# actionml/universal-recommender

Measured on AMD Instinct MI355X. Metric: cooccurrence pairs/sec (A'A+A'B) + LLR top-k items/sec, higher is better.
Workload: dtype int32 counts / f64 LLR; 1 GPU; config4: synthetic 10M users x 2M items, Zipf-1.0, 5 event types (purchase/view/add-to-cart/search/category-pref); generator=torch Philox on the GPU (universal_recommender_amd.synth.generate_device), maxEventsPerEventType=500, maxCorrelatorsPerEventType=50, seed=20260925, entry_point=urcco_context_build_device (C ABI, include/urcco.h), launch=one process per GPU, parallelism=items range-partitioned over 1 GPU(s), one HIP stream per event type

## Files before the change

### universal-recommender_amd/csrc/cco_expand.hip

```cpp
#include "cco_kernels.h"

#include <atomic>
#include <cstdio>
#include <cstdlib>

#include "cco_common.h"
#include "cco_device.h"


namespace urcco {

__global__ __launch_bounds__(256) void item_entropy_kernel(const int32_t* __restrict__ counts, int32_t n, long long n_users,
                                                           double* __restrict__ ent, double* __restrict__ xlx_n) {
  const int64_t i = (int64_t)blockIdx.x * 256 + threadIdx.x;
  if (i < n) {
    const long long c = counts[i];
    ent[i] = entropy2(c, n_users - c);
  }
  if (i == 0 && xlx_n) *xlx_n = x_log_x(n_users);
}

hipError_t launch_item_entropy(hipStream_t st, const int32_t* counts, int32_t n, long long n_users, double* ent, double* xlx_n) {
  const int blocks = n > 0 ? (n + 255) / 256 : 1;
  hipLaunchKernelGGL(item_entropy_kernel, dim3(blocks), dim3(256), 0, st, counts, n, n_users, ent, xlx_n);
  return hipGetLastError();
}

__global__ __launch_bounds__(256) void narrow_counts_kernel(const int32_t* __restrict__ counts, int64_t n, unsigned short* __restrict__ out16,
                                                            int32_t* __restrict__ bad) {
  int over = 0;
  for (int64_t i = (int64_t)blockIdx.x * 256 + threadIdx.x; i < n; i += (int64_t)gridDim.x * 256) {
    const int c = counts[i];
    out16[i] = (unsigned short)c;
    over += (c < 0 || c > 0xffff) ? 1 : 0;
  }
  if (over) atomicAdd(bad, over);
}
hipError_t launch_narrow_counts(hipStream_t st, int n_cu, const int32_t* counts, int64_t n, unsigned short* out16, int32_t* bad) {
  hipError_t e = hipMemsetAsync(bad, 0, sizeof(int32_t), st);
  if (e != hipSuccess || n <= 0) return e;
  int64_t blocks = (n + 255) / 256;
  if (blocks > (int64_t)n_cu * 8) blocks = (int64_t)n_cu * 8;
  hipLaunchKernelGGL(narrow_counts_kernel, dim3((unsigned)blocks), dim3(256), 0, st, counts, n, out16, bad);
  return hipGetLastError();
}

typedef int urcco_v4i __attribute__((ext_vector_type(4)));
// ... 400 lines not shown
```

### universal-recommender_amd/csrc/cco_kernels.h

```cpp
#pragma once
#include <hip/hip_runtime.h>
#include <stdint.h>

namespace urcco {

constexpr int NBINS = 7;
constexpr int MP_KMAX_HOST = 256;

constexpr int SCAN_TILE = 2048;
constexpr int DS_TILE = 4096;
constexpr int GLOBAL_BIN_BLOCKS = 128;
constexpr int BIN_TILE = 1024;
constexpr int XLX_TABLE_HOST = 4096;
constexpr int BIN_COLS_HOST = 3 * NBINS + 3;
constexpr int BIN_OFF_LEN = NBINS + 3;
constexpr int CAND_SLOTS = 64;
constexpr int STATS_LEN = 32;

constexpr int32_t DBG_GATHER_ONLY = 1;
constexpr int32_t DBG_NO_LLR = 2;
constexpr int32_t DBG_NO_TOPK = 4;
constexpr int32_t DBG_NO_SELECT = 8;
constexpr int32_t DBG_NO_RANK = 16;
constexpr int32_t DBG_NO_COUNT_GATHER = 512;
constexpr int32_t DBG_UNFUSED_EXPAND = 4096;
constexpr int32_t DBG_GATHERED_PRIMARY = 8192;
constexpr int32_t DBG_UNFILTERED_EXCHANGE = 16384;
constexpr int32_t DBG_SELECT_DELAY = 131072;
constexpr int32_t DBG_UNPACKED_COUNTS = 1048576;
constexpr int32_t DBG_ROW_KERNELS = DBG_GATHER_ONLY | DBG_NO_LLR | DBG_NO_TOPK | DBG_NO_SELECT | DBG_NO_RANK | DBG_NO_COUNT_GATHER | DBG_SELECT_DELAY;

constexpr int32_t FORM_WIDE = 1;
constexpr int32_t FORM_PS64 = 2;
constexpr int32_t FORM_TILE = 4;
constexpr int32_t FORM_PACK = 8;
constexpr int32_t FORM_HOST = 16;
constexpr unsigned long long NARROW_LIMIT = 1ull << 32;
struct ExpandForm {
  int32_t* word;
  const int32_t* pack_bad;
  int32_t host_wide;
  int32_t host_narrow;
  unsigned long long limit;
  long long seed;
};

struct CcoArgs {
  const int32_t* bin_rows;
  const int32_t* bin_off;
  const int64_t* a_col_ptr;
  const unsigned* pstart32;
  const int64_t* wp;
// ... 14 lines not shown
  int32_t debug;
  long long n_users;
  int32_t n_cols_b;
  int32_t item_lo;
  int32_t exclude_self;
  int32_t k;
  int32_t has_min_llr;
  double min_llr;
  int32_t count_bits;
  int32_t col_bytes;
  int32_t g_log2;
  int32_t unordered;
  int32_t* out_count;
  int32_t* out_idx;
  double* out_llr;
  unsigned long long* err;
  unsigned long long* cand;
  int32_t* g_counts;
  unsigned long long* g_cand_key;
  int32_t* g_cand_col;
  int32_t g_blocks;
  const int64_t* pstart64;
  const int64_t* work;
};

hipError_t launch_column_counts(hipStream_t st, int n_cu, const int32_t* col_idx, int64_t nnz, int32_t n_cols, int32_t* counts);
constexpr int64_t PH_MIN_NNZ = 1 << 20;
int64_t column_counts_scratch_bytes(int64_t nnz, int32_t n_cols);
hipError_t launch_column_counts_partitioned(hipStream_t st, const int32_t* col_idx, int64_t nnz, const int64_t* nnz_dev, int32_t n_cols,
                                            int32_t* counts, char* scratch);

hipError_t launch_scan_i32(hipStream_t st, const int32_t* in, int64_t n, int64_t* out, int64_t* tile_sums);
hipError_t launch_slice_weights(hipStream_t st, const unsigned short* loc_t, int n_buckets, int64_t n_parts, long long* weight);

hipError_t launch_downsample_flags(hipStream_t st, int n_cu, int64_t n_rows, const int64_t* row_ptr, const int32_t* col_idx, int64_t nnz,
                                   int32_t n_cols, const int32_t* raw_counts, unsigned long long* thresholds, uint32_t seed, int32_t max_n,
                                   int row_rate_mode, int64_t row_base, int64_t* tile_rows, unsigned long long* flags, int64_t* tile_count,
                                   int32_t* post_counts);
hipError_t launch_downsample_scan(hipStream_t st, int64_t nnz, int64_t* tile_count);
hipError_t launch_downsample_compact(hipStream_t st, int64_t n_rows, const int64_t* row_ptr, const int32_t* col_idx, int64_t nnz,
                                     const int64_t* tile_rows, const unsigned long long* flags, const int64_t* tile_off, int64_t* out_row_ptr,
                                     int32_t* out_col_idx);

hipError_t launch_scan_i32_range(hipStream_t st, const int32_t* in, int64_t n, int32_t lo, int32_t hi, int64_t* out, int64_t* tile_sums);
hipError_t launch_transpose(hipStream_t st, int n_cu, int64_t n_rows, const int64_t* row_ptr, const int32_t* col_idx, int g_log2,
                            const int64_t* col_ptr, int32_t* cursor, int32_t* out_row_idx, int32_t col_lo, int32_t col_hi);
// ... 25 lines not shown
hipError_t launch_need_mask(hipStream_t st, int n_cu, int64_t n_rows, const int64_t* a_row_ptr, const int32_t* a_col_idx, const int32_t* bounds, int world,
                            unsigned long long* mask);
hipError_t launch_masked_lengths(hipStream_t st, int n_cu, int64_t n_rows, const int64_t* row_ptr, const unsigned long long* mask, int world, int32_t* mlen, int64_t* off,
                                 int64_t* tile_sums, int64_t* to_nnz);
hipError_t launch_pack_rows(hipStream_t st, int n_cu, int64_t n_rows, const int64_t* row_ptr, const int32_t* col_idx, const unsigned long long* mask, int world,
                            const int64_t* off, int32_t* pack);
hipError_t launch_scan_u16(hipStream_t st, const unsigned short* in, int64_t n, int64_t* out, int64_t* tile_sums);
hipError_t launch_frag_record(hipStream_t st, int32_t world, const int32_t* bounds, const int64_t* l_cp, const int32_t* bad, int64_t* rec);
hipError_t launch_frag_place(hipStream_t st, int n_cu, int32_t world, int32_t lo, int32_t n_range, const void* lens, int wire16, const int64_t* src_off,
                             const int32_t* ents, const int64_t* a_cp, const int64_t* sizes, int32_t* a_ri);

hipError_t launch_validate_csr(hipStream_t st, int n_cu, int64_t n_rows, const int64_t* row_ptr, const int32_t* col_idx, int64_t nnz, int32_t n_cols,
                               int g_log2, int64_t rp0, unsigned long long* err);
hipError_t launch_rebase_i64(hipStream_t st, int n_cu, int64_t* p, int64_t n, int64_t delta);
hipError_t launch_publish_word(hipStream_t st, const unsigned long long* src, unsigned long long* dst_mapped);

hipError_t launch_pop_counts(hipStream_t st, int n_cu, int64_t n, const int32_t* item, const int64_t* t_ms, int32_t n_items, int n_buckets,
                             const int64_t* bounds, int32_t* counts);

hipError_t launch_pack_counts(hipStream_t st, int n_cu, const int32_t* col_idx, const int64_t* nnz_dev, int64_t nnz_bound, const unsigned short* counts16,
                              const int32_t* bad16, int32_t count_bits, int32_t* out, int32_t* bad);
hipError_t launch_xlx_table(hipStream_t st, double* tab);
hipError_t launch_xlx_hi_table(hipStream_t st, double* tab , const double* xlx_tab, long long n_users);
hipError_t launch_item_entropy(hipStream_t st, const int32_t* counts, int32_t n, long long n_users, double* ent, double* xlx_n);
hipError_t launch_narrow_counts(hipStream_t st, int n_cu, const int32_t* counts, int64_t n, unsigned short* out16, int32_t* bad);

hipError_t launch_expand_prepare(hipStream_t st, int n_cu, const int64_t* a_col_ptr, int32_t n_items_a, const int32_t* a_row_idx,
                                 const int64_t* b_row_ptr, unsigned* b_rp32_scratch , int64_t n_rows_b, int64_t cap,
                                 unsigned* pstart32, int64_t* pstart64, int32_t* plen, int64_t* wp, int64_t* tile_sums, ExpandForm form);
constexpr int EXPAND_MULTI_MAX = 8;
hipError_t launch_expand_prepare_multi(hipStream_t st, int n_cu, const int64_t* a_col_ptr, int32_t n_items_a, const int32_t* a_row_idx, int n,
                                       const int64_t* const* b_row_ptr, int64_t n_rows_b, int64_t cap, unsigned* const* pstart, int32_t* const* plen, void* T,
                                       int64_t* const* tsum );
hipError_t launch_expand_scan(hipStream_t st, const int64_t* a_col_ptr, int32_t n_items_a, const int32_t* plen, int64_t cap, int64_t* wp, int64_t* tile_sums,
                              bool tile_sums_ready, const unsigned* pstart32, int64_t* pstart64, ExpandForm form);
hipError_t launch_row_work(hipStream_t st, int n_cu, int32_t item_lo, int32_t item_hi, const int64_t* a_col_ptr, const int64_t* wp, const int64_t* tile_sums,
                           const int32_t* form, int64_t* work);

hipError_t launch_binning(hipStream_t st, int32_t item_lo, int32_t n, const int64_t* work, const int32_t* cnt_a, int32_t n_cols_b,
                          int32_t count_bits, int32_t k, int64_t* tile_counts, int32_t* bin_off, int32_t* bin_rows, int64_t* stats);

hipError_t launch_cco_rows_bin(hipStream_t st, int n_cu, const CcoArgs& args, int bin, int32_t n_rows );
hipError_t launch_bin_out_stats(hipStream_t st, const int32_t* bin_rows, const int32_t* bin_off, int32_t item_lo, const int32_t* out_count,
                                const unsigned long long* cand, int64_t* stats);

hipError_t launch_compact_indicators(hipStream_t st, int32_t n_rows, int32_t k, const int32_t* count, const int32_t* idx,
                                     const double* llr, const int64_t* row_ptr, int32_t* out_idx, double* out_llr);
// ... 99 lines not shown
```

### universal-recommender_amd/csrc/cco_rows.hip

```cpp
#include "cco_kernels.h"

#include <atomic>
#include <cstdlib>

#include "cco_common.h"
#include "cco_device.h"


namespace urcco {

constexpr int E0 = 1024, E1S = 4096, E1 = 8192, E2S = 16384, E2 = 32768;
constexpr int MP_KMAX = 256;

__host__ __device__ constexpr int table_slots(int E, int T) { return (2 * E / 3) / (2 * T) * (2 * T); }
constexpr int URCCO_WB1 = 512;
constexpr int URCCO_WB2 = 8192;
__device__ __forceinline__ int choose_bin(long long w, long long ca, int32_t n_cols_b, int32_t count_bits, int32_t k) {
  if (ca <= 0 || w <= 0) return -1;
  if (count_bits < 31 && ca > ((1ll << count_bits) - 1)) return NBINS - 1;
  if (w <= 64 && ca <= 64) return 0;
  int cap_bin = NBINS - 1;
  const long long dmax = (w < (long long)n_cols_b ? w : (long long)n_cols_b) * 3 + (long long)k * 3 + 2;
  if (dmax <= E0) cap_bin = 1;
  else if (dmax <= E1S) cap_bin = 2;
// ... 391 lines not shown
template <int T>
__device__ __forceinline__ unsigned claim_positions(bool want, unsigned* counter, unsigned& wave_count) {
  const unsigned long long m = __ballot(want);
  const unsigned c = (unsigned)__popcll(m);
  unsigned base;
  if (T == WAVE) {
    base = wave_count;
    wave_count += c;
  } else {
    unsigned b = 0u;
    if ((threadIdx.x & (WAVE - 1)) == 0 && c != 0u) b = atomicAdd(counter, c);
    base = wave_read_lane(b, 0);
  }
  return base + lanes_below(m);
}
template <int T>
__device__ __forceinline__ unsigned team_exclusive_scan(unsigned v, unsigned* s_wsum , unsigned* total) {
  const int lane = threadIdx.x & (WAVE - 1);
  const unsigned inc = wave_inclusive_sum(v);
  if (T == WAVE) {
    *total = wave_read_lane(inc, WAVE - 1);
    return inc - v;
  }
  const int wave = (threadIdx.x % T) / WAVE;
  if (lane == WAVE - 1) s_wsum[wave] = inc;
  __syncthreads();
  unsigned base = 0, tot = 0;
#pragma unroll
  for (int w = 0; w < T / WAVE; ++w) {
    const unsigned sw = s_wsum[w];
    if (w < wave) base += sw;
    tot += sw;
  }
  __syncthreads();
  *total = tot;
  return base + inc - v;
}

constexpr int URCCO_U_WAVE = 2;
constexpr int URCCO_U_BS = 2;
constexpr int URCCO_U_B = 2;
constexpr int URCCO_U_H = 1;
constexpr int URCCO_U_C = 1;
constexpr int URCCO_OCC_WAVE = 8;
constexpr int URCCO_OCC_BS = 7;
constexpr int URCCO_G_WAVE = 2;
constexpr int URCCO_SEL_AMB_WAVE = 64;
constexpr int URCCO_SEL_AMB_BLOCK = 128;
constexpr int URCCO_G_BLOCK = 2;
constexpr int URCCO_SEL_M_BLOCK = 128;
constexpr int URCCO_G_CU = 2;
template <bool NARROW> struct PStart { typedef int64_t type; };
template <> struct PStart<true> { typedef unsigned type; };
template <int T, int E, int U, bool MP = false, bool DBG = false, bool PK = false>
__global__ __launch_bounds__((T < 256 ? 256 : T), (T == 64 ? URCCO_OCC_WAVE : (T == 256 && E == 4096 ? URCCO_OCC_BS : (T == 512 ? 4 : 1)))) void cco_rows_kernel(CcoArgs a, int bin) {
  if ((a.b_packed != nullptr && (a.pk_known != 0 || *a.form == 0)) != PK) return;
  using PS = typename PStart<PK>::type;
  constexpr int WS = PK ? 1 : 2;
  const int dbg = DBG ? a.debug : 0;
  constexpr bool packed = PK;
  URCCO_OWN_GLOBAL_PTR(const int32_t, b_col_idx, PK ? a.b_packed : a.b_col_idx);
  const int cshift = 32 - a.count_bits;
  const unsigned colmask = PK ? (1u << cshift) - 1u : a.b_col_mask;
  URCCO_OWN_GLOBAL_PTR(const unsigned short, cnt_b16, a.cnt_b16);
  URCCO_OWN_GLOBAL_PTR(const int32_t, cnt_b, a.cnt_b);
  URCCO_OWN_GLOBAL_PTR(const double, xlx_tab, a.xlx_tab);
  URCCO_OWN_GLOBAL_PTR(const double, xlx_hi, a.xlx_hi);
  URCCO_OWN_GLOBAL_PTR(const double, col_ent, a.col_ent);
  URCCO_OWN_GLOBAL_PTR(int32_t, out_idx, a.out_idx);
  URCCO_OWN_GLOBAL_PTR(double, out_llr, a.out_llr);
  long long n_users = a.n_users;
  URCCO_OWN_SGPRS(n_users);
  constexpr int BLOCK = T < 256 ? 256 : T;
  constexpr int TEAMS = BLOCK / T;
  constexpr int SH = table_slots(E, T);
  constexpr int SPT = SH / T;
  static_assert(SH % (2 * T) == 0 && SH + SH / 2 <= E && SH <= 65536, "slots and the candidate list share the table; a slot index takes 16 bits of a list word");
  constexpr unsigned CAND_CAP = (unsigned)(E - SH);
// ... 27 lines not shown
  __shared__ unsigned long long s_selthr[TEAMS * 2];
  constexpr bool SKIP_SHARED = T >= 256;
  __shared__ unsigned long long s_kbits[2 * NW];
  __shared__ unsigned s_mpflag;
  __shared__ unsigned s_ncand;
  __shared__ unsigned long long s_runk[MP ? 2 * MP_KMAX : 1];
  __shared__ unsigned s_runc[MP ? 2 * MP_KMAX : 1];

  const int team = TEAMS == 1 ? 0 : uni((int)threadIdx.x / T);
  const int tl = threadIdx.x % T;
  const int lane = threadIdx.x & (WAVE - 1);
  unsigned* tab = s_tab + team * E;
  unsigned* cand = tab + SH;
  unsigned long long* share = s_share + (SHARE ? team * SHARE_WORDS : 0);
  PS* ustart = reinterpret_cast<PS*>(SHARE ? reinterpret_cast<long long*>(share) : s_ustart + team * T);
  unsigned* uoff = SHARE ? reinterpret_cast<unsigned*>(share + T) : s_uoff + team * (T + 1);
  unsigned* hist = SHARE ? reinterpret_cast<unsigned*>(share) : s_hist + team * NH * 128;
  unsigned* sel_res = s_selres + team * 4;
  unsigned* nsel = sel_res + 3;
  unsigned short* lst = SHARE ? reinterpret_cast<unsigned short*>(share) + SH_LST / 2 : s_lst + team * (SEL_CAP > 0 ? SEL_CAP : 1);
  unsigned long long* amb_key = SHARE ? share : s_ambkey + team * SEL_M;
  unsigned* amb_col = SHARE ? reinterpret_cast<unsigned*>(share + SEL_M) : s_ambcol + team * SEL_M;
  unsigned long long* sel_thr = s_selthr + team * 2;
  const int list_start = a.bin_off[bin];
  const int list_n = a.bin_off[bin + 1] - list_start;
  const int total_teams = gridDim.x * TEAMS;
  bool ident = (long long)a.n_cols_b * 3 + (long long)a.k * 3 + 2 <= E && a.n_cols_b <= SH;
  int cb = a.count_bits;
  unsigned cmask = (1u << cb) - 1u;
  unsigned long long cand_acc = 0ull;
  const double xlx_n = *a.xlx_n;
  const bool use16 = *a.cnt16_bad == 0;

  int li = blockIdx.x * TEAMS + team;
  if (li >= list_n) return;
  const int S = total_teams;
  auto pos_of = [&](int l) { return list_start + (l < list_n ? l : list_n - 1); };
  const unsigned* wp32 = reinterpret_cast<const unsigned*>(a.wp);
  const PS* pstart;
  if constexpr (PK) pstart = a.pstart32;
  else pstart = a.pstart64;
  const int lane3 = lane < 3 ? lane : 2;
  int idv = a.bin_rows[pos_of(li + lane3 * S)];
  int64_t cs_c, ce_c;
  int64_t bnd_b;
  {
// ... 47 lines not shown
        const long long cols_pp = ((long long)a.n_cols_b + (1ll << mp_s) - 1) >> mp_s;
        int kb = 1;
        while ((1ll << kb) <= cols_pp) ++kb;
        const bool count_ok = kb <= 1 || ca_row <= (1ll << (32 - kb)) - 1;
        const long long exp_d = ((dd >> mp_s) + (dd >> (mp_s + 2)) + 1) < cols_pp ? ((dd >> mp_s) + (dd >> (mp_s + 2)) + 1) : cols_pp;
        if (count_ok && exp_d <= cap) break;
      }
    }
  mp_again:
    if (MP) {
      const long long cols_pp = ((long long)a.n_cols_b + (1ll << mp_s) - 1) >> mp_s;
      int kb = 1;
      while ((1ll << kb) <= cols_pp) ++kb;
      cb = 32 - kb;
      cmask = cb >= 32 ? 0xffffffffu : (1u << cb) - 1u;
      ident = cols_pp * 3 + 3ll * a.k + 2ll <= (long long)E && cols_pp <= (long long)SH;
      if (tl == 0) s_mpflag = 0u;
    }
    const unsigned mp_mask = MP ? (1u << mp_s) - 1u : 0u;
#pragma unroll
    for (int q = 0; q < SPT / 2; ++q) *reinterpret_cast<uint2*>(&tab[2 * (tl + q * T)]) = make_uint2(0u, 0u);
    unsigned n_cand = 0u;
    if (T != WAVE && tl == 0) s_ncand = 0u;
    team_sync<T>();
    for (int64_t c0 = cs; c0 < ce; c0 += T) {
      const int64_t c1 = c0 + T < ce ? c0 + T : ce;
      const bool pre = !MP && c0 == cs;
      const unsigned w0 = pre ? row_w0 : uni(wp32[WS * c0]);
      const unsigned total = (pre ? row_w1 : uni(wp32[WS * c1])) - w0;
      const int64_t p = c0 + tl;
      if (p < c1) {
        ustart[tl] = pre ? my_start : pstart[p];
        uoff[tl] = (pre ? my_wp : wp32[WS * p]) - w0;
      } else {
        uoff[tl] = total;
      }
      if (tl == 0) uoff[T] = total;
      team_sync<T>();
      if (total > 0u) {
        const unsigned per = (total + T - 1) / T;
        const unsigned first = (unsigned)tl * per;
        const bool act = first < total;
        const unsigned last = act ? (first + per < total ? first + per : total) : first;
        int o = 0;
        int64_t pos = 0;
        unsigned uend = 0u;
// ... 56 lines not shown
              n_cand += n_new;
            } else {
              unsigned b = 0u;
              if (lane == 0) b = atomicAdd(&s_ncand, n_new);
              base = wave_read_lane(b, 0);
            }
#pragma unroll
            for (int q = 0; q < G; ++q) {
              const unsigned idx = base + lanes_below(cm[q]);
              if (at[q] != ~0u) {
                if (idx < CAND_CAP) cand[idx] = at[q] | ((packed ? jj[q] >> cshift : 0u) << 16);
                else if (MP) s_mpflag = 1u;
                else atomicAdd(a.err, 1ull);
              }
              base += (unsigned)__popcll(cm[q]);
            }
          }
        }
      }
      team_sync<T>();
    }
    unsigned D = T == WAVE ? n_cand : uni(s_ncand);
    if (D > CAND_CAP) D = CAND_CAP;
    {
      unsigned cw[CPT], cv[CPT];
#pragma unroll
      for (int q = 0; q < CPT; ++q) {
        const unsigned t = (unsigned)tl + (unsigned)q * T;
        cw[q] = 0u;
        cv[q] = 0u;
        if (t < D) {
          cw[q] = cand[t];
          cv[q] = tab[cw[q] & 0xffffu];
        }
      }
      team_sync<T>();
      unsigned long long* kk0 = reinterpret_cast<unsigned long long*>(tab + ((D + 1u) & ~1u));
      const bool fits = !MP || 3ll * D + 3ll * a.k + 2ll <= (long long)E;
#pragma unroll
      for (int q = 0; q < CPT; ++q) {
        const unsigned t = (unsigned)tl + (unsigned)q * T;
        if (t < D) {
          tab[t] = cv[q];
          if (fits) kk0[t] = (unsigned long long)(cw[q] >> 16);
        }
      }
    }
    team_sync<T>();
    if (MP) {
      if (s_mpflag != 0u || 3ll * D + 3ll * a.k + 2ll > (long long)E) {
        team_sync<T>();
        ++mp_s;
        mp_q = 0u;
        n_run = 0u;
        goto mp_again;
      }
    }
    cand_acc += D;
    unsigned long long* kk = reinterpret_cast<unsigned long long*>(tab + ((D + 1u) & ~1u));
    unsigned n_valid = 0;
    unsigned long long kand = ~0ull, kor = 0ull;
    {
      const long long ca = a.cnt_a[i];
      const double row_entropy = a.ent_a[i];
      for (unsigned base = 0; base < D; base += U * T) {
        const unsigned t0 = base + (unsigned)tl;
        unsigned vv[U];
        int cbj[U];
// ... 22 lines not shown
            if (!(a.exclude_self && j == i)) {
              const double llr = all_in_tables ? llr_from_tables(row_entropy, xlx_n, (unsigned)k11, (unsigned)ca, (unsigned)cbj[x], xlx_tab, xlx_hi, col_ent)
                                               : ((dbg & DBG_NO_LLR) ? (double)k11
                                                            : llr_of(row_entropy, xlx_n, k11, ca, (long long)cbj[x], n_users, xlx_tab, xlx_hi, col_ent));
              if (llr > 0.0 && (!a.has_min_llr || llr >= a.min_llr)) key = (unsigned long long)__double_as_longlong(llr);
            }
            kk[t] = key;
            if (key != 0ull) {
              ++n_valid;
              if (SKIP_SHARED) {
                kand &= key;
                kor |= key;
              }
            }
          }
        }
      }
    }
    URCCO_SETTLE(idv); URCCO_SETTLE(bnd_c);
    if (!MP) { URCCO_SETTLE(pf_w0); URCCO_SETTLE(pf_w1); URCCO_SETTLE(pf_wp); URCCO_SETTLE(pf_start); }
    if (SKIP_SHARED) {
      wave_and_or_u64(kand, kor);
      if (lane == 0) {
        s_kbits[2 * (tl / WAVE)] = kand;
        s_kbits[2 * (tl / WAVE) + 1] = kor;
      }
    }
    unsigned C;
    team_exclusive_scan<T>(n_valid, s_wsum, &C);
    C = uni(C);
    team_sync<T>();
    const int64_t obase = ((int64_t)(i - a.item_lo)) * a.k;
    unsigned long long thr_key = 0ull;
    unsigned thr_ncol = 0u;
    bool row_done = false;
    if (!(dbg & DBG_NO_TOPK)) {
      if (dbg & DBG_NO_SELECT) {
        if (C > (unsigned)a.k) thr_key = ~0ull;
      } else if (C > (unsigned)a.k) {
        unsigned need = (unsigned)a.k;
        if (a.col_bytes < 4) thr_ncol = 0xffffffffu << (8 * a.col_bytes);
        int p0 = 0;
        if (!SKIP_SHARED) {
          kand = ~0ull;
          kor = 0ull;
          for (unsigned base = 0; base < D; base += T) {
            const unsigned t = base + (unsigned)tl;
            const unsigned long long key = t < D ? kk[t] : 0ull;
// ... 726 lines not shown
#pragma unroll
      for (int w2 = 0; w2 < NW; ++w2) {
        const unsigned long long ok = s_pkey[r & 1][w2];
        const int oc = s_pcol[r & 1][w2];
        if (best_before(ok, oc, wk, wc)) {
          wk = ok;
          wc = oc;
        }
      }
      if (wk == 0ull) break;
      if (threadIdx.x == 0) {
        a.out_idx[obase + r] = wc;
        a.out_llr[obase + r] = __longlong_as_double((long long)wk);
      }
      last_key = wk;
      last_col = wc;
      ++emitted;
    }
    if (threadIdx.x == 0) a.out_count[i - a.item_lo] = emitted;
    __syncthreads();
  }
}

static int blocks_per_cu(int bin) {
  static std::atomic<int> cache[7];
  if (cache[bin].load(std::memory_order_relaxed) == 0) {
    int n = 0;
    hipError_t e = hipErrorUnknown;
    if (bin == 0) e = hipOccupancyMaxActiveBlocksPerMultiprocessor(&n, (cco_rows_micro_kernel<WAVE, false, false>), 256, 0);
    if (bin == 1) e = hipOccupancyMaxActiveBlocksPerMultiprocessor(&n, cco_rows_kernel<64, E0, URCCO_U_WAVE>, 256, 0);
    if (bin == 2) e = hipOccupancyMaxActiveBlocksPerMultiprocessor(&n, cco_rows_kernel<256, E1S, URCCO_U_BS>, 256, 0);
    if (bin == 3) e = hipOccupancyMaxActiveBlocksPerMultiprocessor(&n, cco_rows_kernel<256, E1, URCCO_U_B>, 256, 0);
    if (bin == 4) e = hipOccupancyMaxActiveBlocksPerMultiprocessor(&n, cco_rows_kernel<512, E2S, URCCO_U_H>, 512, 0);
    if (bin == 5) e = hipOccupancyMaxActiveBlocksPerMultiprocessor(&n, cco_rows_kernel<1024, E2, URCCO_U_C>, 1024, 0);
    if (bin == 6) e = hipOccupancyMaxActiveBlocksPerMultiprocessor(&n, cco_rows_kernel<1024, E2, URCCO_U_C, true>, 1024, 0);
    cache[bin].store((e == hipSuccess && n > 0) ? n : 1, std::memory_order_relaxed);
  }
  return cache[bin].load(std::memory_order_relaxed);
}

hipError_t launch_cco_rows_bin(hipStream_t st, int n_cu, const CcoArgs& args, int bin, int32_t n_rows) {
  static constexpr int factor[NBINS] = {8, 8, 8, 8, 4, 4, 2};
  constexpr int micro_factor32 = 3, micro_factor16 = 2;
  auto grid = [&](int b, int f = 0) {
    const long long fill = (long long)n_cu * blocks_per_cu(b);
    const long long teams = b <= 1 ? 4 : 1;
    long long cap = ((long long)n_rows + teams * 32 - 1) / (teams * 32);
    if (cap < 2 * fill) cap = 2 * fill;
    long long blocks = fill * (f > 0 ? f : factor[b]);
    if (blocks > cap) blocks = cap;
    return dim3((unsigned)blocks);
  };
  const bool dbgk = (args.debug & DBG_ROW_KERNELS) != 0;
  CcoArgs plain = args;
  plain.b_packed = nullptr;
  const bool both = args.b_packed != nullptr && !dbgk && !args.pk_known;
#define URCCO_LAUNCH_ROWS(TT, EE, UU, MPF, GRID, BLK, BINARG)                                                                      \
  do {                                                                                                                           \
    if (dbgk) hipLaunchKernelGGL((cco_rows_kernel<TT, EE, UU, MPF, true, false>), GRID, dim3(BLK), 0, st, plain, BINARG);          \
    else {                                                                                                                       \
      if (both || args.pk_known) hipLaunchKernelGGL((cco_rows_kernel<TT, EE, UU, MPF, false, true>), GRID, dim3(BLK), 0, st, args, BINARG); \
      if (!args.pk_known) hipLaunchKernelGGL((cco_rows_kernel<TT, EE, UU, MPF, false, false>), GRID, dim3(BLK), 0, st, args, BINARG); \
    }                                                                                                                            \
  } while (0)
#define URCCO_LAUNCH_MICRO(LL, GRID)                                                                                  \
  do {                                                                                                                \
    if (dbgk) hipLaunchKernelGGL((cco_rows_micro_kernel<LL, true, false>), GRID, dim3(256), 0, st, plain);              \
    else {                                                                                                            \
      if (both || args.pk_known) hipLaunchKernelGGL((cco_rows_micro_kernel<LL, false, true>), GRID, dim3(256), 0, st, args); \
      if (!args.pk_known) hipLaunchKernelGGL((cco_rows_micro_kernel<LL, false, false>), GRID, dim3(256), 0, st, args);  \
    }                                                                                                                 \
  } while (0)
  switch (bin) {
    case 0:
      URCCO_LAUNCH_MICRO(64, grid(0));
      if (micro_split_for(n_rows)) {
        URCCO_LAUNCH_MICRO(32, grid(0, micro_factor32));
        URCCO_LAUNCH_MICRO(16, grid(0, micro_factor16));
      }
      break;
    case 1: URCCO_LAUNCH_ROWS(64, E0, URCCO_U_WAVE, false, grid(1), 256, 1); break;
    case 2: URCCO_LAUNCH_ROWS(256, E1S, URCCO_U_BS, false, grid(2), 256, 2); break;
    case 3: URCCO_LAUNCH_ROWS(256, E1, URCCO_U_B, false, grid(3), 256, 3); break;
    case 4: URCCO_LAUNCH_ROWS(512, E2S, URCCO_U_H, false, grid(4), 512, 4); break;
// ... 36 lines not shown
```

### universal-recommender_amd/csrc/urcco_api.hip

```cpp
#include "urcco_internal.h"

using namespace urcco_detail;

#include <signal.h>
#include <unistd.h>

#include <mutex>

namespace urcco_detail {
char* err_buf() {
  static thread_local char buf[512] = "";
  return buf;
}

const DebugCfg& debug_cfg() {
  static const DebugCfg cfg = [] {
    DebugCfg c;
    const char* m = getenv("URCCO_DEBUG_MARKS");
    const char* p = getenv("URCCO_DEBUG_POISON");
    c.marks = m && *m && *m != '0';
    c.poison = p && *p && *p != '0';
    return c;
  }();
  return cfg;
// ... 400 lines not shown
  if (!s || item_lo < 0 || item_hi < item_lo || item_hi > n_items_a || n_cols_b < 0 || n_users < 0 || nnz_a_bound < 0 || !a_col_ptr || !b_row_ptr)
    return fail(URCCO_BAD_ARG, "urcco_dev_cco_rows: bad argument");
  if (k <= 0) return fail(URCCO_BAD_ARG, "maxInterestingElements must be positive, got %d", k);
  const int32_t n = item_hi - item_lo;
  if (n == 0) {
    if (stats_dev) HIPC(hipMemsetAsync(stats_dev, 0, sizeof(int64_t) * URCCO_STATS_LEN, s->stream));
    return URCCO_OK;
  }
  if (!out_count || !out_idx || !out_llr || !counts_a || (n_cols_b > 0 && !counts_b)) return fail(URCCO_BAD_ARG, "urcco_dev_cco_rows: NULL buffer");
  HIPC(hipMemsetAsync(out_count, 0, sizeof(int32_t) * (size_t)n, s->stream));
  if (n_cols_b == 0 || n_users == 0) {
    if (stats_dev) HIPC(hipMemsetAsync(stats_dev, 0, sizeof(int64_t) * URCCO_STATS_LEN, s->stream));
    return URCCO_OK;
  }
  int key_bits = 0;
  URC(packed_key_bits(n_cols_b, &key_bits));
  const int count_bits = 32 - key_bits;
  const bool dense_bin6 = k > urcco::MP_KMAX_HOST || 3ll * k + 5 > 32768ll;
  if (dense_bin6) URC(s->ensure_global_bin(n_cols_b));
  if (!s->xlx_tab.p) {
    URC(s->xlx_tab.alloc(urcco::XLX_TABLE_HOST));
    HIPC(urcco::launch_xlx_table(s->stream, s->xlx_tab.p));
  }
  if (!s->xlx_hi.p) URC(s->xlx_hi.alloc(2 * urcco::XLX_TABLE_HOST));
  if (s->xlx_hi_n != n_users) {
    HIPC(urcco::launch_xlx_hi_table(s->stream, s->xlx_hi.p, s->xlx_tab.p, n_users));
    s->xlx_hi_n = n_users;
  }
  const int64_t n_tiles = ((int64_t)n + urcco::BIN_TILE - 1) / urcco::BIN_TILE;
  const int64_t cap = nnz_a_bound;
  if (!s->form_word.p) URC(s->form_word.alloc(1));
  s->form_valid = false;
  ArenaLayout L(s);
  int64_t *pstart64, *wp, *p_tile_sums, *work, *tile_counts, *stats = stats_dev;
  unsigned *own_pstart = nullptr, *b_rp32;
  int32_t *own_plen, *bin_off, *bin_rows, *cnt16_bad;
  double *ent_a, *xlx_n;
  unsigned short* cnt_b16;
  unsigned long long* cand;
  L.add(&pstart64, (size_t)cap);
  if (!pre_pstart) L.add(&own_pstart, (size_t)cap);
  L.add(&own_plen, (size_t)cap).add(&wp, (size_t)cap + 1).add(&p_tile_sums, scan_tile_words(cap));
  L.add(&work, (size_t)n).add(&tile_counts, (size_t)(n_tiles + 1) * urcco::BIN_COLS_HOST);
  L.add(&bin_off, urcco::BIN_OFF_LEN).add(&bin_rows, (size_t)n);
  L.add(&ent_a, (size_t)n_items_a).add(&cnt_b16, (size_t)n_cols_b).add(&cnt16_bad, 1);
  L.add(&cand, urcco::CAND_SLOTS).add(&xlx_n, 1);
  if (!stats_dev) L.add(&stats, URCCO_STATS_LEN);
  L.add(&b_rp32, (size_t)n_users + 1);
  URC(L.commit());
  const unsigned* pstart32 = pre_pstart ? pre_pstart : own_pstart;
  int32_t* form = s->form_word.p;

  const int32_t* packed = pk_known ? b_col_idx : ((b_packed && pack_bad && !(s->debug & urcco::DBG_UNPACKED_COUNTS)) ? b_packed : nullptr);
  const bool host_wide = packed == nullptr || (s->debug & urcco::DBG_ROW_KERNELS) != 0;
  const bool narrow_known = pk_known && !host_wide && b_nnz_bound >= 0 && b_nnz_bound < ((int64_t)1 << 32) &&
                            (unsigned long long)n_cols_b * (unsigned long long)urcco::SCAN_TILE < s->narrow_limit;
  const urcco::ExpandForm ef{form, pk_known ? nullptr : pack_bad, host_wide ? 1 : 0, narrow_known ? 1 : 0, s->narrow_limit, s->prefix_seed};
  int64_t* tile_sums = (pre_pstart && pre_plen && pre_tile_sums) ? pre_tile_sums : p_tile_sums;
  s->begin(URCCO_STAGE_ROW_WORK);
  if (pre_pstart && pre_plen)
    HIPC(urcco::launch_expand_scan(s->stream, a_col_ptr, n_items_a, pre_plen, cap, wp, tile_sums, pre_tile_sums != nullptr, pre_pstart, pstart64, ef));
  else
    HIPC(urcco::launch_expand_prepare(s->stream, s->n_cu, a_col_ptr, n_items_a, a_row_idx, b_row_ptr, b_rp32, n_users, cap, own_pstart, pstart64, own_plen, wp, tile_sums, ef));
  HIPC(urcco::launch_row_work(s->stream, s->n_cu, item_lo, item_hi, a_col_ptr, wp, tile_sums, form, work));
  s->form_valid = true;
  s->end();
  s->begin(URCCO_STAGE_BINNING);
  HIPC(hipMemsetAsync(stats, 0, sizeof(int64_t) * URCCO_STATS_LEN, s->stream));
  HIPC(urcco::launch_binning(s->stream, item_lo, n, work, counts_a, n_cols_b, count_bits, k, tile_counts, bin_off, bin_rows, stats));
  s->end();
  s->begin(URCCO_STAGE_ENTROPY);
  HIPC(urcco::launch_item_entropy(s->stream, counts_a, n_items_a, n_users, ent_a, xlx_n));
  HIPC(urcco::launch_narrow_counts(s->stream, s->n_cu, counts_b, n_cols_b, cnt_b16, cnt16_bad));
  s->end();

  urcco::CcoArgs a;
  a.bin_rows = bin_rows; a.bin_off = bin_off;
  a.a_col_ptr = a_col_ptr; a.pstart32 = pstart32; a.pstart64 = pstart64; a.wp = wp; a.form = form; a.work = work; a.b_col_idx = b_col_idx;
  a.b_packed = packed; a.pk_known = narrow_known ? 1 : 0;
  a.b_col_mask = pk_known ? (key_bits >= 32 ? 0xffffffffu : (1u << key_bits) - 1u) : 0xffffffffu;
  a.cnt_a = counts_a; a.cnt_b = counts_b; a.ent_a = ent_a; a.cnt_b16 = cnt_b16; a.cnt16_bad = cnt16_bad; a.xlx_n = xlx_n; a.xlx_tab = s->xlx_tab.p; a.xlx_hi = s->xlx_hi.p; a.col_ent = s->xlx_hi.p + urcco::XLX_TABLE_HOST; a.debug = s->debug;
  a.n_users = n_users; a.n_cols_b = n_cols_b; a.item_lo = item_lo; a.exclude_self = exclude_self ? 1 : 0; a.k = k;
  a.has_min_llr = has_min_llr ? 1 : 0; a.min_llr = min_llr; a.count_bits = count_bits;
  a.col_bytes = n_cols_b <= (1 << 8) ? 1 : (n_cols_b <= (1 << 16) ? 2 : (n_cols_b <= (1 << 24) ? 3 : 4));
  a.unordered = s->unordered_rows ? 1 : 0;
  a.g_log2 = 4;
  a.out_count = out_count; a.out_idx = out_idx; a.out_llr = out_llr;
  a.err = reinterpret_cast<unsigned long long*>(stats + 1 + 4 * urcco::NBINS);
  a.cand = s->timing ? cand : nullptr;
  if (s->timing) HIPC(hipMemsetAsync(cand, 0, sizeof(unsigned long long) * urcco::CAND_SLOTS, s->stream));
  a.g_counts = s->g_counts.p; a.g_cand_key = s->g_cand_key.p; a.g_cand_col = s->g_cand_col.p; a.g_blocks = dense_bin6 ? s->g_blocks : 0;
  for (int step = 0; step < urcco::NBINS; ++step) {
    const int bin = urcco::NBINS - 1 - step;
    s->begin(URCCO_STAGE_CCO_BIN0 + bin);
    HIPC(urcco::launch_cco_rows_bin(s->stream, s->n_cu, a, bin, n));
    s->end();
  }
  if (s->timing) HIPC(urcco::launch_bin_out_stats(s->stream, bin_rows, bin_off, item_lo, out_count, cand, stats));
  return URCCO_OK;
}

int pack_counts(urcco_session* s, const int64_t* b_row_ptr, int64_t n_rows_b, const int32_t* b_col_idx, int64_t nnz_bound, const int32_t* counts_b, int32_t n_cols_b,
                int32_t* out, int32_t* bad) {
  if (!s || !b_row_ptr || n_rows_b < 0 || nnz_bound < 0 || !out || !bad || (nnz_bound > 0 && (!b_col_idx || !counts_b))) return fail(URCCO_BAD_ARG, "pack_counts: bad argument");
// ... 364 lines not shown
```

Measured before the change: 35.09 billion pairs/s.

## Prefilter count-1 candidates using per-row LLR monotonicity limit before top-k

Precomputes, for each row count, the column-count range over which LLR with co-count 1 is strictly decreasing in the column count, and stores a per-item limit alongside the entropy pass. In the large-row cco kernels, a shared histogram of count-1 candidates by column count finds the cutoff where k candidates are guaranteed better, then compacts away dominated count-1 candidates before LLR scoring and top-k selection. This cuts LLR evaluations and selection work on long rows, at the cost of an extra histogram, scan, and compaction pass, plus extra shared memory use.

```diff
diff --git a/universal-recommender_amd/csrc/cco_expand.hip b/universal-recommender_amd/csrc/cco_expand.hip
--- a/universal-recommender_amd/csrc/cco_expand.hip
+++ b/universal-recommender_amd/csrc/cco_expand.hip
@@ -11,18 +11,21 @@
 namespace urcco {
 
 __global__ __launch_bounds__(256) void item_entropy_kernel(const int32_t* __restrict__ counts, int32_t n, long long n_users,
-                                                           double* __restrict__ ent, double* __restrict__ xlx_n) {
+                                                           double* __restrict__ ent, double* __restrict__ xlx_n, const unsigned short* __restrict__ mono,
+                                                           unsigned short* __restrict__ lim) {
   const int64_t i = (int64_t)blockIdx.x * 256 + threadIdx.x;
   if (i < n) {
     const long long c = counts[i];
     ent[i] = entropy2(c, n_users - c);
+    if (mono) lim[i] = (c >= 0 && c < (long long)XLX_TABLE) ? mono[c] : (unsigned short)0;
   }
   if (i == 0 && xlx_n) *xlx_n = x_log_x(n_users);
 }
 
-hipError_t launch_item_entropy(hipStream_t st, const int32_t* counts, int32_t n, long long n_users, double* ent, double* xlx_n) {
+hipError_t launch_item_entropy(hipStream_t st, const int32_t* counts, int32_t n, long long n_users, double* ent, double* xlx_n, const unsigned short* mono,
+                               unsigned short* lim) {
   const int blocks = n > 0 ? (n + 255) / 256 : 1;
-  hipLaunchKernelGGL(item_entropy_kernel, dim3(blocks), dim3(256), 0, st, counts, n, n_users, ent, xlx_n);
+  hipLaunchKernelGGL(item_entropy_kernel, dim3(blocks), dim3(256), 0, st, counts, n, n_users, ent, xlx_n, lim ? mono : nullptr, lim);
   return hipGetLastError();
 }
 
diff --git a/universal-recommender_amd/csrc/cco_kernels.h b/universal-recommender_amd/csrc/cco_kernels.h
--- a/universal-recommender_amd/csrc/cco_kernels.h
+++ b/universal-recommender_amd/csrc/cco_kernels.h
@@ -28,6 +28,8 @@
 constexpr int32_t DBG_UNFILTERED_EXCHANGE = 16384;
 constexpr int32_t DBG_SELECT_DELAY = 131072;
 constexpr int32_t DBG_UNPACKED_COUNTS = 1048576;
+constexpr int32_t DBG_NO_PREFILTER = 8388608;
+constexpr int32_t DBG_COUNT_SCORED = 16777216;
 constexpr int32_t DBG_ROW_KERNELS = DBG_GATHER_ONLY | DBG_NO_LLR | DBG_NO_TOPK | DBG_NO_SELECT | DBG_NO_RANK | DBG_NO_COUNT_GATHER | DBG_SELECT_DELAY;
 
 constexpr int32_t FORM_WIDE = 1;
@@ -88,6 +90,7 @@
   int32_t g_blocks;
   const int64_t* pstart64;
   const int64_t* work;
+  const unsigned short* pf_limit;
 };
 
 hipError_t launch_column_counts(hipStream_t st, int n_cu, const int32_t* col_idx, int64_t nnz, int32_t n_cols, int32_t* counts);
@@ -159,7 +162,9 @@
                               const int32_t* bad16, int32_t count_bits, int32_t* out, int32_t* bad);
 hipError_t launch_xlx_table(hipStream_t st, double* tab);
 hipError_t launch_xlx_hi_table(hipStream_t st, double* tab , const double* xlx_tab, long long n_users);
-hipError_t launch_item_entropy(hipStream_t st, const int32_t* counts, int32_t n, long long n_users, double* ent, double* xlx_n);
+hipError_t launch_item_entropy(hipStream_t st, const int32_t* counts, int32_t n, long long n_users, double* ent, double* xlx_n, const unsigned short* mono = nullptr,
+                               unsigned short* lim = nullptr);
+hipError_t launch_mono_limit(hipStream_t st, unsigned short* mono, const double* xlx_tab, const double* hi_tab, long long n_users);
 hipError_t launch_narrow_counts(hipStream_t st, int n_cu, const int32_t* counts, int64_t n, unsigned short* out16, int32_t* bad);
 
 hipError_t launch_expand_prepare(hipStream_t st, int n_cu, const int64_t* a_col_ptr, int32_t n_items_a, const int32_t* a_row_idx,
diff --git a/universal-recommender_amd/csrc/cco_rows.hip b/universal-recommender_amd/csrc/cco_rows.hip
--- a/universal-recommender_amd/csrc/cco_rows.hip
+++ b/universal-recommender_amd/csrc/cco_rows.hip
@@ -437,7 +437,9 @@
     *total = wave_read_lane(inc, WAVE - 1);
     return inc - v;
   }
-  const int wave = (threadIdx.x % T) / WAVE;
+  int tz = (int)threadIdx.x;
+  URCCO_OPAQUE(tz);
+  const int wave = (tz % T) / WAVE;
   if (lane == WAVE - 1) s_wsum[wave] = inc;
   __syncthreads();
   unsigned base = 0, tot = 0;
@@ -465,10 +467,13 @@
 constexpr int URCCO_G_BLOCK = 2;
 constexpr int URCCO_SEL_M_BLOCK = 128;
 constexpr int URCCO_G_CU = 2;
+__host__ __device__ constexpr bool prefilter_class(int T, int E) { return T >= WAVE && E >= 1024; }
+constexpr unsigned PF_BINS = 256;
 template <bool NARROW> struct PStart { typedef int64_t type; };
 template <> struct PStart<true> { typedef unsigned type; };
 template <int T, int E, int U, bool MP = false, bool DBG = false, bool PK = false>
-__global__ __launch_bounds__((T < 256 ? 256 : T), (T == 64 ? URCCO_OCC_WAVE : (T == 256 && E == 4096 ? URCCO_OCC_BS : (T == 512 ? 4 : 1)))) void cco_rows_kernel(CcoArgs a, int bin) {
+__global__ __launch_bounds__((T < 256 ? 256 : T), (T == 64 ? URCCO_OCC_WAVE : (T == 256 && E == 4096 ? URCCO_OCC_BS : (T == 512 ? 4 : 1)))) void cco_rows_kernel(CcoArgs a, int bin_arg) {
+  const int bin = bin_arg & 255;
   if ((a.b_packed != nullptr && (a.pk_known != 0 || *a.form == 0)) != PK) return;
   using PS = typename PStart<PK>::type;
   constexpr int WS = PK ? 1 : 2;
@@ -542,6 +547,9 @@
   unsigned long long* amb_key = SHARE ? share : s_ambkey + team * SEL_M;
   unsigned* amb_col = SHARE ? reinterpret_cast<unsigned*>(share + SEL_M) : s_ambcol + team * SEL_M;
   unsigned long long* sel_thr = s_selthr + team * 2;
+  constexpr bool PF = PK && !MP && prefilter_class(T, E);
+  static_assert(!PF || !SHARE || T == WAVE || (sizeof(PS) == 4 && T * 4 + PF_BINS * 2 <= T * 8), "the histogram sits behind the 32-bit starts");
+  unsigned* pfh = (SHARE && T != WAVE) ? reinterpret_cast<unsigned*>(share) + T : hist;
   const int list_start = a.bin_off[bin];
   const int list_n = a.bin_off[bin + 1] - list_start;
   const int total_teams = gridDim.x * TEAMS;
@@ -635,6 +643,11 @@
     for (int q = 0; q < SPT / 2; ++q) *reinterpret_cast<uint2*>(&tab[2 * (tl + q * T)]) = make_uint2(0u, 0u);
     unsigned n_cand = 0u;
     if (T != WAVE && tl == 0) s_ncand = 0u;
+    if (PF && T != WAVE) {
+      int tz = tl;
+      URCCO_OPAQUE(tz);
+      if (tz < (int)PF_BINS / 2) pfh[tz] = 0u;
+    }
     team_sync<T>();
     for (int64_t c0 = cs; c0 < ce; c0 += T) {
       const int64_t c1 = c0 + T < ce ? c0 + T : ce;
@@ -737,6 +750,10 @@
     }
     unsigned D = T == WAVE ? n_cand : uni(s_ncand);
     if (D > CAND_CAP) D = CAND_CAP;
+    unsigned pf_lim = 0u;
+    if (PF) {
+      if (T == WAVE) *reinterpret_cast<uint2*>(&pfh[2 * lane]) = make_uint2(0u, 0u);
+    }
     {
       unsigned cw[CPT], cv[CPT];
 #pragma unroll
@@ -749,7 +766,59 @@
           cv[q] = tab[cw[q] & 0xffffu];
         }
       }
+      const unsigned pf_need = (unsigned)a.k + (a.exclude_self ? 1u : 0u);
+      const bool pf_try = PF && a.pf_limit != nullptr && D > pf_need;
+      if (PF && pf_try) {
+#pragma unroll
+        for (int q = 0; q < CPT; ++q) {
+          const unsigned cbq = cw[q] >> 16;
+          if ((cv[q] & cmask) == 1u && cbq < PF_BINS - 1u) atomicAdd(&pfh[cbq >> 1], 1u << (16 * (cbq & 1u)));
+        }
+      }
       team_sync<T>();
+      bool pf_cut = false;
+      unsigned cstar = 0u, lim = 0u;
+      if (PF && pf_try) {
+        pf_lim = (unsigned)a.pf_limit[i];
+        int lq = lane;
+        URCCO_OPAQUE(lq);
+        const unsigned w01 = pfh[2 * lq], w23 = pfh[2 * lq + 1];
+        const unsigned h0 = w01 & 0xffffu, h1 = w01 >> 16, h2 = w23 & 0xffffu, h3 = w23 >> 16;
+        const unsigned v4 = h0 + h1 + h2 + h3;
+        const unsigned S = wave_inclusive_sum(v4);
+        const unsigned long long ge = __ballot(S >= pf_need);
+        const int L = ge != 0ull ? __ffsll((unsigned long long)ge) - 1 : 0;
+        const unsigned below = S - v4;
+        const unsigned d = below + h0 >= pf_need ? 0u : (below + h0 + h1 >= pf_need ? 1u : (below + h0 + h1 + h2 >= pf_need ? 2u : 3u));
+        cstar = wave_read_lane(4u * (unsigned)lq + d, L);
+        lim = uni(pf_lim);
+        pf_cut = ge != 0ull && cstar < lim;
+      }
+      if (PF && pf_cut) {
+        unsigned cnt = 0u;
+#pragma unroll
+        for (int q = 0; q < CPT; ++q) {
+          const unsigned t = (unsigned)tl + (unsigned)q * T;
+          const unsigned cbq = cw[q] >> 16;
+          const bool drop = (cv[q] & cmask) == 1u && cbq > cstar && cbq <= lim;
+          if (t < D && !drop) ++cnt;
+          else cv[q] = 0u;
+        }
+        unsigned Dn;
+        unsigned pos = team_exclusive_scan<T>(cnt, s_wsum, &Dn);
+        Dn = uni(Dn);
+        unsigned long long* kkn = reinterpret_cast<unsigned long long*>(tab + ((Dn + 1u) & ~1u));
+#pragma unroll
+        for (int q = 0; q < CPT; ++q) {
+          if (cv[q] != 0u) {
+            tab[pos] = cv[q];
+            kkn[pos] = (unsigned long long)(cw[q] >> 16);
+            ++pos;
+          }
+        }
+        if (!(bin_arg & 256)) cand_acc += D - Dn;
+        D = Dn;
+      } else {
       unsigned long long* kk0 = reinterpret_cast<unsigned long long*>(tab + ((D + 1u) & ~1u));
       const bool fits = !MP || 3ll * D + 3ll * a.k + 2ll <= (long long)E;
 #pragma unroll
@@ -759,6 +828,7 @@
           tab[t] = cv[q];
           if (fits) kk0[t] = (unsigned long long)(cw[q] >> 16);
         }
+      }
       }
     }
     team_sync<T>();
@@ -827,8 +897,10 @@
     if (SKIP_SHARED) {
       wave_and_or_u64(kand, kor);
       if (lane == 0) {
-        s_kbits[2 * (tl / WAVE)] = kand;
-        s_kbits[2 * (tl / WAVE) + 1] = kor;
+        int tw = tl;
+        URCCO_OPAQUE(tw);
+        s_kbits[2 * (tw / WAVE)] = kand;
+        s_kbits[2 * (tw / WAVE) + 1] = kor;
       }
     }
     unsigned C;
@@ -1601,6 +1673,34 @@
   }
 }
 
+__global__ __launch_bounds__(256) void mono_limit_kernel(unsigned short* __restrict__ mono, const double* __restrict__ xlx_tab, const double* __restrict__ xlx_hi,
+                                                         const double* __restrict__ col_ent, long long n_users) {
+  __shared__ unsigned s_min;
+  const unsigned ca = blockIdx.x;
+  if (threadIdx.x == 0) s_min = (unsigned)XLX_TABLE;
+  __syncthreads();
+  const double xlx_n = x_log_x(n_users);
+  const double row_entropy = (long long)ca <= n_users ? entropy2((long long)ca, n_users - (long long)ca) : 0.0;
+  for (unsigned cb = 1u + threadIdx.x; cb < (unsigned)XLX_TABLE; cb += 256u) {
+    bool ok = llr_operands_in_tables(1u, (long long)ca, cb, n_users, col_ent) && llr_operands_in_tables(1u, (long long)ca, cb + 1u, n_users, col_ent);
+    if (ok) {
+      const double f0 = llr_from_tables(row_entropy, xlx_n, 1u, ca, cb, xlx_tab, xlx_hi, col_ent);
+      const double f1 = llr_from_tables(row_entropy, xlx_n, 1u, ca, cb + 1u, xlx_tab, xlx_hi, col_ent);
+      ok = f0 > f1 && f0 > 0.0;
+    }
+    if (!ok) {
+      atomicMin(&s_min, cb);
+      break;
+    }
+  }
+  __syncthreads();
+  if (threadIdx.x == 0) mono[ca] = (unsigned short)(s_min <= 1u ? 0u : s_min);
+}
+hipError_t launch_mono_limit(hipStream_t st, unsigned short* mono, const double* xlx_tab, const double* hi_tab , long long n_users) {
+  hipLaunchKernelGGL(mono_limit_kernel, dim3(XLX_TABLE), dim3(256), 0, st, mono, xlx_tab, hi_tab, hi_tab + XLX_TABLE, n_users);
+  return hipGetLastError();
+}
+
 static int blocks_per_cu(int bin) {
   static std::atomic<int> cache[7];
   if (cache[bin].load(std::memory_order_relaxed) == 0) {
@@ -1631,6 +1731,7 @@
     return dim3((unsigned)blocks);
   };
   const bool dbgk = (args.debug & DBG_ROW_KERNELS) != 0;
+  const int scored = (args.debug & DBG_COUNT_SCORED) ? 256 : 0;
   CcoArgs plain = args;
   plain.b_packed = nullptr;
   const bool both = args.b_packed != nullptr && !dbgk && !args.pk_known;
@@ -1638,7 +1739,7 @@
   do {                                                                                                                           \
     if (dbgk) hipLaunchKernelGGL((cco_rows_kernel<TT, EE, UU, MPF, true, false>), GRID, dim3(BLK), 0, st, plain, BINARG);          \
     else {                                                                                                                       \
-      if (both || args.pk_known) hipLaunchKernelGGL((cco_rows_kernel<TT, EE, UU, MPF, false, true>), GRID, dim3(BLK), 0, st, args, BINARG); \
+      if (both || args.pk_known) hipLaunchKernelGGL((cco_rows_kernel<TT, EE, UU, MPF, false, true>), GRID, dim3(BLK), 0, st, args, BINARG | scored); \
       if (!args.pk_known) hipLaunchKernelGGL((cco_rows_kernel<TT, EE, UU, MPF, false, false>), GRID, dim3(BLK), 0, st, args, BINARG); \
     }                                                                                                                            \
   } while (0)
diff --git a/universal-recommender_amd/csrc/urcco_api.hip b/universal-recommender_amd/csrc/urcco_api.hip
--- a/universal-recommender_amd/csrc/urcco_api.hip
+++ b/universal-recommender_amd/csrc/urcco_api.hip
@@ -446,9 +446,11 @@
     URC(s->xlx_tab.alloc(urcco::XLX_TABLE_HOST));
     HIPC(urcco::launch_xlx_table(s->stream, s->xlx_tab.p));
   }
-  if (!s->xlx_hi.p) URC(s->xlx_hi.alloc(2 * urcco::XLX_TABLE_HOST));
+  if (!s->xlx_hi.p) URC(s->xlx_hi.alloc(2 * urcco::XLX_TABLE_HOST + urcco::XLX_TABLE_HOST / 4));
+  unsigned short* mono = reinterpret_cast<unsigned short*>(s->xlx_hi.p + 2 * urcco::XLX_TABLE_HOST);
   if (s->xlx_hi_n != n_users) {
     HIPC(urcco::launch_xlx_hi_table(s->stream, s->xlx_hi.p, s->xlx_tab.p, n_users));
+    HIPC(urcco::launch_mono_limit(s->stream, mono, s->xlx_tab.p, s->xlx_hi.p, n_users));
     s->xlx_hi_n = n_users;
   }
   const int64_t n_tiles = ((int64_t)n + urcco::BIN_TILE - 1) / urcco::BIN_TILE;
@@ -460,14 +462,14 @@
   unsigned *own_pstart = nullptr, *b_rp32;
   int32_t *own_plen, *bin_off, *bin_rows, *cnt16_bad;
   double *ent_a, *xlx_n;
-  unsigned short* cnt_b16;
+  unsigned short *cnt_b16, *pf_limit;
   unsigned long long* cand;
   L.add(&pstart64, (size_t)cap);
   if (!pre_pstart) L.add(&own_pstart, (size_t)cap);
   L.add(&own_plen, (size_t)cap).add(&wp, (size_t)cap + 1).add(&p_tile_sums, scan_tile_words(cap));
   L.add(&work, (size_t)n).add(&tile_counts, (size_t)(n_tiles + 1) * urcco::BIN_COLS_HOST);
   L.add(&bin_off, urcco::BIN_OFF_LEN).add(&bin_rows, (size_t)n);
-  L.add(&ent_a, (size_t)n_items_a).add(&cnt_b16, (size_t)n_cols_b).add(&cnt16_bad, 1);
+  L.add(&ent_a, (size_t)n_items_a).add(&cnt_b16, (size_t)n_cols_b).add(&cnt16_bad, 1).add(&pf_limit, (size_t)n_items_a);
   L.add(&cand, urcco::CAND_SLOTS).add(&xlx_n, 1);
   if (!stats_dev) L.add(&stats, URCCO_STATS_LEN);
   L.add(&b_rp32, (size_t)n_users + 1);
@@ -494,7 +496,7 @@
   HIPC(urcco::launch_binning(s->stream, item_lo, n, work, counts_a, n_cols_b, count_bits, k, tile_counts, bin_off, bin_rows, stats));
   s->end();
   s->begin(URCCO_STAGE_ENTROPY);
-  HIPC(urcco::launch_item_entropy(s->stream, counts_a, n_items_a, n_users, ent_a, xlx_n));
+  HIPC(urcco::launch_item_entropy(s->stream, counts_a, n_items_a, n_users, ent_a, xlx_n, mono, pf_limit));
   HIPC(urcco::launch_narrow_counts(s->stream, s->n_cu, counts_b, n_cols_b, cnt_b16, cnt16_bad));
   s->end();
 
@@ -504,6 +506,7 @@
   a.b_packed = packed; a.pk_known = narrow_known ? 1 : 0;
   a.b_col_mask = pk_known ? (key_bits >= 32 ? 0xffffffffu : (1u << key_bits) - 1u) : 0xffffffffu;
   a.cnt_a = counts_a; a.cnt_b = counts_b; a.ent_a = ent_a; a.cnt_b16 = cnt_b16; a.cnt16_bad = cnt16_bad; a.xlx_n = xlx_n; a.xlx_tab = s->xlx_tab.p; a.xlx_hi = s->xlx_hi.p; a.col_ent = s->xlx_hi.p + urcco::XLX_TABLE_HOST; a.debug = s->debug;
+  a.pf_limit = (s->debug & urcco::DBG_NO_PREFILTER) ? nullptr : pf_limit;
   a.n_users = n_users; a.n_cols_b = n_cols_b; a.item_lo = item_lo; a.exclude_self = exclude_self ? 1 : 0; a.k = k;
   a.has_min_llr = has_min_llr ? 1 : 0; a.min_llr = min_llr; a.count_bits = count_bits;
   a.col_bytes = n_cols_b <= (1 << 8) ? 1 : (n_cols_b <= (1 << 16) ? 2 : (n_cols_b <= (1 << 24) ? 3 : 4));
```

Result: faster. 38.38 billion pairs/s, median of 6 (+9.4%).
